# TencentARC/TVTS

Measured on AMD Instinct MI355X. Metric: video-text pairs/sec/node, TVTSv2 pretrain step, higher is better.
Workload: dtype bf16; 1 GPU; TVTSv2 ViT-B/16 8-frame 224^2, mask 0.5, 32-token captions x4, full pretrain step (fwd+losses+bwd+HF-AdamW); pairs_per_gpu=192, global_batch=192, parallelism=dp1, hip_graph=False

## Files before the change

include/tvts_hip.h:

```cpp
#ifndef TVTS_HIP_H
#define TVTS_HIP_H
#include <hip/hip_runtime_api.h>
#ifdef __cplusplus
extern "C" {
#endif

enum { TVTS_ACT_NONE = 0, TVTS_ACT_QUICK_GELU = 1, TVTS_ACT_GELU_ERF = 2,
       TVTS_GATE_ADD_BF16 = 3  };
enum { TVTS_ATTN_FULL = 0, TVTS_ATTN_SPACE = 1, TVTS_ATTN_TIME = 2, TVTS_ATTN_CLS = 3 };
enum {
    TVTS_GEMM_TILE_128 = 1,
    TVTS_GEMM_TILE_256 = 2,
    TVTS_GEMM_FP8_K32 = 4,
    TVTS_TN_NO_EARLY_DMA = 4,
    TVTS_TN_AFAST_0 = 8,
    TVTS_TN_AFAST_1 = 16,
    TVTS_GEMM_STREAMK = 32,
    TVTS_GEMM_NO_STREAMK = 64,
    TVTS_GEMM_RING = 128,
    TVTS_GEMM_NO_RING = 16384,
    TVTS_GEMM_F32_PATCH = 4194304,
    TVTS_GEMM_CLOCK_SAMPLE = 2097152,
    TVTS_GEMM_SIDE_DERIV = 1048576
};
#define TVTS_GEMM_RING_ROWS(r) ((r) == 128 ? (1 << 16) : (r) == 192 ? (2 << 16) : (r) == 256 ? (3 << 16) : 0)
#define TVTS_GEMM_CUS(n) ((((n) / 8) & 63) << 8)
#define TVTS_TN_SPLITS(s) ((s) << 8)
enum {
    TVTS_ATTN_NO_TR = 1,
    TVTS_ATTN_NO_SHARED = 2,
    TVTS_ATTN_NO_FUSED = 4
};

int tvts_gemm_nt_bf16(const void* A, int lda, const void* B, int ldb, int M, int N, int K, const float* bias,
                      const float* residual, int ldr, int act, void* preact, int ldp, const void* gate_h, int ldh,
                      int gate_act, void* out, int ldc, int out_f32, void* workspace, long workspace_bytes, int opts,
                      hipStream_t stream);
long tvts_gemm_nt_workspace_bytes(void);
int tvts_gemm_nt_select(int M, int N, int opts);
int tvts_gemm_tn_bf16(const void* P, int ldp, const void* Q, int ldq, int M, int Na, int Nb, float* out, int ldo,
                      int accumulate, float* colsum, float* workspace, long workspace_elems, int* counters, int n_counters,
                      int opts, hipStream_t stream);
int tvts_gemm_tn_bf16_grouped(const void* problems, int n, void* table_dev, void* table_host, long table_bytes, int upload,
                              float* workspace, long workspace_elems, int opts, hipStream_t stream);
long tvts_gemm_tn_grouped_table_bytes(int n);
int tvts_gemm_tn_select(int M, int Na, int Nb, int opts);
int tvts_gemm_nt_fp8(const void* A, int lda, const void* B, int ldb, int M, int N, int K, const float* scale_a,
                     int scale_a_rows, const float* scale_b, const float* bias, const float* residual, int ldr, int act, void* preact, int ldp,
                     void* out, int ldc, int out_f32, void* q8out, int ldq8, const float* q8_scale, float* q8_amax, int opts,
                     hipStream_t stream);
int tvts_gemm_nt_fp8_gate(const void* A, int lda, const void* B, int ldb, int M, int N, int K, const float* scale_a,
                          int scale_a_rows, const float* scale_b, const float* bias, const void* gate_h, int ldh, int gate_act,
                          void* out, int ldc, void* q8out, int ldq8, const float* q8_scale, float* q8_amax, int opts,
                          hipStream_t stream);
int tvts_gemm_tn_fp8(const void* P8, int ldp, const void* Q8, int ldq, int M, int Na, int Nb, const float* scale_p,
                     const float* scale_q, float* out, int ldo, int accumulate, float* colsum, float* workspace,
                     long workspace_elems, int opts, hipStream_t stream);
int tvts_amax(const void* x, int is_f32, long ld, int rows, int cols, float* amax, hipStream_t stream);
int tvts_quant_fp8(const void* x, int is_f32, long ld, int rows, int cols, const float* amax, void* out, long ldo,
                   float* scale_out, hipStream_t stream);
int tvts_quant_fp8_multi(const void* table, int n, hipStream_t stream);
int tvts_quant_fp8_rows(const void* x, long ld, int rows, int cols, void* out, long ldo, float* row_scale,
                        const float* tscale, float* amax_acc, hipStream_t stream);
int tvts_fp8_update_scales(float* amax, float* scale, int n, hipStream_t stream);
int tvts_gemm_small_f32(const float* A, long sai, long sak, const float* B, long sbk, long sbj, int M, int N, int K,
                        float alpha, const float* bias, float* C, long ldc, int accumulate, hipStream_t stream);
int tvts_rows_linear_bf16(const void* A, long lda, const void* W, int ldw, int R, int N, int K, const float* bias, const float* residual,
                          int ldr, float* out, int ldo, hipStream_t stream);
// ... 187 lines not shown
```

tvts_amd/csrc/gemm.hip:

```cpp
#include "common.h"
#include <stdlib.h>
#include <type_traits>

#include "gemm_nt256.h"

#define BM 128
#define BN 128
#define NTHREADS 256

__device__ __forceinline__ void stage_rows128(const bf16* __restrict__ base, int ld, int row0, int row_max,
                                              int k0, char* lds_tile, int wave, int lane) {
#pragma unroll
    for (int t = 0; t < 4; ++t) {
        const int r0 = (t * 4 + wave) * 8;
        const int row = r0 + (lane >> 3);
        const int slot = lane & 7;
        const int chunk = slot ^ (row & 7);
        int grow = row0 + row;
        grow = grow < row_max ? grow : row_max;
        const bf16* src = base + (size_t)grow * ld + k0 + chunk * 8;
        __builtin_amdgcn_global_load_lds((const GLB_PTR(void))src, (LDS_PTR(void))(lds_tile + r0 * 128), 16, 0, 0);
    }
}

// ... 857 lines not shown
    const int grid = ceil_div(g.n_items, 8) * 8;
    if (t256) {
        hipError_t e2 = hipFuncSetAttribute((const void*)gemm_tn256_kernel, hipFuncAttributeMaxDynamicSharedMemorySize, 131072);
        if (e2 != hipSuccess) return (int)e2;
        hipLaunchKernelGGL(gemm_tn256_kernel, dim3(grid), dim3(512), 131072, stream, g);
    } else {
        hipError_t e2 = hipFuncSetAttribute((const void*)gemm_tn_kernel, hipFuncAttributeMaxDynamicSharedMemorySize, 65536);
        if (e2 != hipSuccess) return (int)e2;
        hipLaunchKernelGGL(gemm_tn_kernel, dim3(grid), dim3(NTHREADS), 65536, stream, g);
    }
    if (use_ws && !fused) {
        const long n4 = (long)Na * Nb / 4;
        int rb = (int)((n4 + 255) / 256);
        if (rb > 2048) rb = 2048;
        hipLaunchKernelGGL(tn_reduce_kernel, dim3(rb), dim3(256), 0, stream, workspace, splits, Na, Nb, out, ldo, accumulate,
                           g.cs_ws, colsum);
    }
    TVTS_LAUNCH_CHECK();
    return TVTS_OK;
}

struct tvts_tn_problem_ { const void* P; int ldp; const void* Q; int ldq; int M, Na, Nb; float* out; int ldo; int accumulate; float* colsum; };
extern "C" long tvts_gemm_tn_grouped_table_bytes(int n) { return (long)n * (long)sizeof(GemmTN) + (long)(n + 1) * 4 + 64; }
extern "C" int tvts_gemm_tn_bf16_grouped(const void* problems, int n, void* table_dev, void* table_host, long table_bytes, int upload,
                                         float* workspace, long workspace_elems, int opts, hipStream_t stream) {
    if (n <= 0 || n > 64 || !problems || !table_dev || !workspace || table_bytes < tvts_gemm_tn_grouped_table_bytes(n)) return TVTS_EINVAL;
    if (upload && !table_host) return TVTS_EINVAL;
    const tvts_tn_problem_* pr = (const tvts_tn_problem_*)problems;
    GemmTN tab_local[64];
    int prefix_local[65];
    GemmTN* tab = upload ? (GemmTN*)table_host : tab_local;
    int* prefix = upload ? (int*)((char*)table_host + (size_t)n * sizeof(GemmTN)) : prefix_local;
    long tiles_total = 0, out_total = 0;
    int Mmax = 0;
    for (int i = 0; i < n; ++i) {
        if (pr[i].M <= 0 || pr[i].Na % 8 || pr[i].Nb % 8 || pr[i].ldp % 8 || pr[i].ldq % 8 || pr[i].ldo % 4 || pr[i].Nb % 4) return TVTS_EINVAL;
        tiles_total += (long)ceil_div(pr[i].Na, 128) * ceil_div(pr[i].Nb, 128);
        out_total += (long)pr[i].Na * pr[i].Nb;
        Mmax = pr[i].M > Mmax ? pr[i].M : Mmax;
    }
    int sp_best = 1;
    if ((opts >> 8) > 0) {
        sp_best = opts >> 8;
    } else {
        double best = 1e30;
        for (int sp = 1; sp <= 32; ++sp) {
            if (sp > 1 && Mmax / sp < 512) break;
            if (sp > 1 && (double)sp * ((double)out_total + 4096.0 * n) > (double)workspace_elems) break;
            const double rounds = (double)((tiles_total * sp + 511) / 512);
            const double t = rounds * (ceil_div(ceil_div(Mmax, sp), 64) * 64.0) * 0.0148 + (sp > 1 ? sp * (double)out_total * 1e-6 : 0.0);
            if (t < best) { best = t; sp_best = sp; }
        }
    }
    float* ws = workspace;
    long used = 0;
    prefix[0] = 0;
    for (int i = 0; i < n; ++i) {
        GemmTN& g = tab[i];
        const tvts_tn_problem_& q = pr[i];
        g.P = (const bf16*)q.P; g.ldp = q.ldp; g.Q = (const bf16*)q.Q; g.ldq = q.ldq; g.M = q.M; g.Na = q.Na; g.Nb = q.Nb;
        g.out = q.out; g.ldo = q.ldo; g.colsum = q.colsum; g.accumulate = q.accumulate; g.cnt = nullptr;
        g.tiles_a = ceil_div(q.Na, 128); g.tiles_b = ceil_div(q.Nb, 128); g.tiles_ab = g.tiles_a * g.tiles_b;
        g.a_fast = g.tiles_a < g.tiles_b ? 1 : 0;
        g.early_dma = ((unsigned long long)q.M * (unsigned long long)(q.ldp > q.ldq ? q.ldp : q.ldq) * 2ull < (1ull << 32)) ? 1 : 0;
        int splits = sp_best;
        while (splits > 1 && q.M / splits < 256) --splits;
        g.m_per_split = ceil_div(ceil_div(q.M, splits), 64) * 64;
        splits = ceil_div(q.M, g.m_per_split);
        g.splits = splits;
        g.ws = nullptr; g.cs_ws = nullptr;
        if (splits > 1) {
            const long need = (long)splits * q.Na * q.Nb + (q.colsum ? (long)splits * q.Na : 0);
            if (used + need > workspace_elems) return TVTS_EINVAL;
            g.ws = ws + used;
            if (q.colsum) g.cs_ws = ws + used + (long)splits * q.Na * q.Nb;
            used += (need + 63) / 64 * 64;
        }
        g.atomic = (q.accumulate || splits > 1) ? 1 : 0;
        g.n_items = g.tiles_ab * splits;
        prefix[i + 1] = prefix[i] + g.n_items;
        if (splits == 1 && !q.accumulate) {  }
    }
    char* td = (char*)table_dev;
    if (upload) {
        hipError_t e = hipMemcpyAsync(td, table_host, (size_t)n * sizeof(GemmTN) + (size_t)(n + 1) * 4, hipMemcpyHostToDevice, stream);
        if (e != hipSuccess) return (int)e;
    }
    TnGroup grp;
    grp.tab = (const GemmTN*)td; grp.prefix = (const int*)(td + (size_t)n * sizeof(GemmTN)); grp.n = n;
    const int grid = ceil_div(prefix[n], 8) * 8;
    hipError_t e2 = hipFuncSetAttribute((const void*)gemm_tn_grouped_kernel, hipFuncAttributeMaxDynamicSharedMemorySize, 65536);
    if (e2 != hipSuccess) return (int)e2;
    hipLaunchKernelGGL(gemm_tn_grouped_kernel, dim3(grid), dim3(NTHREADS), 65536, stream, grp);
    bool any_ws = false;
    for (int i = 0; i < n; ++i) any_ws = any_ws || tab[i].ws != nullptr;
    if (any_ws) hipLaunchKernelGGL(tn_reduce_grouped_kernel, dim3(384, n), dim3(256), 0, stream, grp);
    TVTS_LAUNCH_CHECK();
    return TVTS_OK;
}

#include "gemm_tn8.h"

extern "C" int tvts_gemm_tn_fp8(const void* P8, int ldp, const void* Q8, int ldq, int M, int Na, int Nb, const float* scale_p,
                                const float* scale_q, float* out, int ldo, int accumulate, float* colsum, float* workspace,
                                long workspace_elems, int opts, hipStream_t stream) {
    if (M <= 0 || Na <= 0 || Nb <= 0 || !scale_p || !scale_q) return TVTS_EINVAL;
    if (Na % 16 || Nb % 16 || ldp % 16 || ldq % 16 || ldo % 4) return TVTS_EINVAL;
    if ((unsigned long long)M * (unsigned long long)(ldp > ldq ? ldp : ldq) >= (1ull << 32)) return TVTS_EINVAL;
    GemmTN8 g;
    g.P = (const unsigned char*)P8; g.ldp = ldp; g.Q = (const unsigned char*)Q8; g.ldq = ldq; g.M = M; g.Na = Na; g.Nb = Nb;
    g.out = out; g.ldo = ldo; g.sp = scale_p; g.sq = scale_q; g.accumulate = accumulate; g.ws = nullptr;
    g.colsum = colsum; g.cs_ws = nullptr;
    g.tiles_a = ceil_div(Na, 256); g.tiles_b = ceil_div(Nb, 256); g.tiles_ab = g.tiles_a * g.tiles_b;
    g.a_fast = g.tiles_a < g.tiles_b ? 1 : 0;
    int splits = 1;
    if ((opts >> 8) > 0) {
// ... 349 lines not shown
```

tvts_amd/csrc/gemm_tn256.h:

```cpp
#pragma once

__device__ __forceinline__ unsigned tn_frag_off(int ct, int lane) {
    const int g = lane >> 4, i = lane & 15;
    const int row = g * 4 + (i >> 2);
    return (unsigned)(row * 256 + ((ct ^ (row & 7)) << 5) + (i & 3) * 8);
}
#ifndef TN_STAGGER_DMA
#define TN_STAGGER_DMA 1
#endif
#ifndef TN_ABL
#define TN_ABL 0
#endif
__device__ __forceinline__ bf16x8 tn_frag(const char* tile, unsigned off, int u) {
    typedef __attribute__((ext_vector_type(8))) short s16x8;
    if (TN_ABL & 2) return *(const bf16x8*)(tile + ((off + u * 8192) & ~15u));
    const s16x4 h0 = __builtin_amdgcn_ds_read_tr16_b64_v4i16((LDS_PTR(s16x4))(tile + off + u * 8192));
    const s16x4 h1 = __builtin_amdgcn_ds_read_tr16_b64_v4i16((LDS_PTR(s16x4))(tile + off + u * 8192 + 4096));
    const s16x8 both = __builtin_shufflevector(h0, h1, 0, 1, 2, 3, 4, 5, 6, 7);
    return __builtin_bit_cast(bf16x8, both);
}
__device__ __forceinline__ void tn_mask(bf16x8& f, int u, int valid, int lane) {
    typedef __attribute__((ext_vector_type(4))) unsigned u32x4;
    const int gq = lane >> 4;
    u32x4 w = __builtin_bit_cast(u32x4, f);
// ... 19 lines not shown
                                                       unsigned lds_stage, int wave, int lane) {
    asm volatile("" : "+v"(lane));
#pragma unroll
    for (int q = 0; q < 8; ++q) {
        const int tile = q >> 1;
        const int r0 = ((q & 1) * 8 + wave) * 4;
        const int row = r0 + (lane >> 4);
        const int s16 = lane & 15;
        const int chunk32 = (s16 >> 1) ^ (row & 7);
        const bool isP = tile < 2;
        const int c0 = (isP ? a0 : b0) + (tile & 1) * 128;
        const int cmax = (isP ? g.Na : g.Nb) - 8;
        int col = c0 + chunk32 * 16 + (s16 & 1) * 8;
        col = col < cmax ? col : cmax;
        int gm = m_stage + row;
        gm = gm < g.M - 1 ? gm : g.M - 1;
        const unsigned off = ((unsigned)(gm - m_stage) * (unsigned)(isP ? g.ldp : g.ldq) + (unsigned)col) * 2u;
        glds16_asm(off, isP ? baseP : baseQ, lds_stage + (unsigned)tile * 16384u + (unsigned)r0 * 256u);
    }
}

__global__ __launch_bounds__(512, 2) void gemm_tn256_kernel(GemmTN g) {
    extern __shared__ __attribute__((aligned(16))) char smem[];
    const int tid = threadIdx.x;
    const int lane = tid & 63;
    const int wave = __builtin_amdgcn_readfirstlane(tid >> 6);
    const int wa = wave >> 2, wb = wave & 3;

    const int xcd = blockIdx.x & 7, jx = blockIdx.x >> 3, per = gridDim.x >> 3;
    const int item = xcd * per + jx;
    if (item >= g.n_items) return;
    const int split = item / g.tiles_ab;
    const int t = item % g.tiles_ab;
    const int ta = g.a_fast ? t % g.tiles_a : t / g.tiles_b, tb = g.a_fast ? t / g.tiles_a : t % g.tiles_b;
    const int a0 = ta * 256, b0 = tb * 256;
    const int m_begin = split * g.m_per_split;
    int m_end = m_begin + g.m_per_split;
    m_end = m_end < g.M ? m_end : g.M;
    if (m_begin >= m_end) return;
    const int nk = (m_end - m_begin + 63) / 64;
    const bool do_cs = g.colsum != nullptr && tb == 0;

    const unsigned lds0 = (unsigned)(size_t)(LDS_PTR(char))smem;
    const char* baseP = (const char*)g.P + (size_t)m_begin * g.ldp * 2;
    const char* baseQ = (const char*)g.Q + (size_t)m_begin * g.ldq * 2;
    const size_t stepP = (size_t)64 * g.ldp * 2, stepQ = (size_t)64 * g.ldq * 2;
    const int row_l = wave * 4 + (lane >> 4), s16_l = lane & 15;
    const int col_l = (((s16_l >> 1) ^ (row_l & 7)) << 4) + (s16_l & 1) * 8;
    const unsigned offP = ((unsigned)row_l * (unsigned)g.ldp + (unsigned)(a0 + col_l)) * 2u;
    const unsigned offQ = ((unsigned)row_l * (unsigned)g.ldq + (unsigned)(b0 + col_l)) * 2u;
    const bool cols_inside = a0 + 256 <= g.Na && b0 + 256 <= g.Nb;
    const size_t halfP = (size_t)32 * g.ldp * 2, halfQ = (size_t)32 * g.ldq * 2;
    int i_st = 0;
    auto issue = [&]() {
        const int m_stage = m_begin + i_st * 64;
        const unsigned dst = lds0 + (unsigned)(i_st & 1) * 65536u + (unsigned)wave * 1024u;
        const char* bp = baseP + ((TN_ABL & 4) ? 0 : (size_t)i_st * stepP);
        const char* bq = baseQ + ((TN_ABL & 4) ? 0 : (size_t)i_st * stepQ);
        if (cols_inside && m_stage + 64 <= g.M) {
            glds16_asm_imm<0>(offP, bp, dst);
            glds16_asm_imm<0>(offP, bp + halfP, dst + 8192u);
            glds16_asm_imm<256>(offP, bp, dst + 16384u);
            glds16_asm_imm<256>(offP, bp + halfP, dst + 16384u + 8192u);
            glds16_asm_imm<0>(offQ, bq, dst + 32768u);
            glds16_asm_imm<0>(offQ, bq + halfQ, dst + 32768u + 8192u);
            glds16_asm_imm<256>(offQ, bq, dst + 49152u);
            glds16_asm_imm<256>(offQ, bq + halfQ, dst + 49152u + 8192u);
        } else {
            tn_stage_issue_clamped(g, a0, b0, m_stage, bp, bq, lds0 + (unsigned)(i_st & 1) * 65536u, wave, lane);
        }
        ++i_st;
    };
    issue();
    asm volatile("s_waitcnt vmcnt(0)" ::: "memory");
    RAW_BARRIER_P();
    if (i_st < nk) issue();

    f32x4 acc[8][4];
#pragma unroll
    for (int i = 0; i < 8; ++i)
#pragma unroll
        for (int j = 0; j < 4; ++j) acc[i][j] = (f32x4){0.f, 0.f, 0.f, 0.f};
    float cs0 = 0.f, cs1 = 0.f;

    const unsigned off0 = tn_frag_off(0, lane);
    const unsigned pBase = (unsigned)wa * 16384u, qBase = 32768u + (unsigned)(wb >> 1) * 16384u;
    const unsigned qOff0 = off0 ^ ((unsigned)(wb & 1) << 7);
#define pOff(ct) (pBase + (off0 ^ ((unsigned)(ct) << 5)))
#define qOff(j) (qBase + (qOff0 ^ ((unsigned)(j) << 5)))

    bf16x8 pF[2][4], qF[2][4];
#define TN_LOAD_P(dst, buf, u, h, valid)                                                               \
    _Pragma("unroll") for (int i = 0; i < 4; ++i) {                                                    \
        dst[i] = tn_frag(buf, pOff((h) * 4 + i), u);                                                   \
        if (TAIL && (valid) < 64) tn_mask(dst[i], u, valid, lane);                                     \
    }
#define TN_LOAD_Q(dst, buf, u) _Pragma("unroll") for (int j = 0; j < 4; ++j) dst[j] = tn_frag(buf, qOff(j), u)
#define TN_MFMA16(pv, qv, h)                                                                           \
    _Pragma("unroll") for (int i = 0; i < 4; ++i)                                                      \
        _Pragma("unroll") for (int j = 0; j < 4; ++j)                                                  \
            acc[(h) * 4 + i][j] = __builtin_amdgcn_mfma_f32_16x16x32_bf16(qv[j], pv[i], acc[(h) * 4 + i][j], 0, 0, 0)
#define TN_CS1(acc_, frag_)                                                                            \
    {                                                                                                  \
        typedef __attribute__((ext_vector_type(2))) __bf16 bf16x2_;                                    \
        typedef __attribute__((ext_vector_type(4))) unsigned u32x4_;                                   \
        const u32x4_ w_ = __builtin_bit_cast(u32x4_, frag_);                                           \
        const bf16x2_ one_ = {(bf16)1.0f, (bf16)1.0f};                                                 \
        _Pragma("unroll") for (int d = 0; d < 4; ++d) {                                                \
            const unsigned wd_ = w_[d];                                                                \
            acc_ = __builtin_amdgcn_fdot2_f32_bf16(__builtin_bit_cast(bf16x2_, wd_), one_, acc_, false); \
        }                                                                                              \
    }
#define TN_CS(pv, h)                                                                                   \
    if (CS && (wb >> 1) == (h)) {                                                                      \
        if (wb & 1) { TN_CS1(cs0, pv[2]) TN_CS1(cs1, pv[3]) }                                          \
        else        { TN_CS1(cs0, pv[0]) TN_CS1(cs1, pv[1]) }                                          \
    }
    int valid = m_end - m_begin;
    {
        constexpr bool TAIL = true;
        TN_LOAD_Q(qF[0], smem, 0);
        TN_LOAD_P(pF[0], smem, 0, 0, valid);
    }
#define TN_STAGE()                                                                                     \
    {                                                                                                  \
        const char* cur = smem + (st & 1) * 65536;                                                     \
        const char* nxt = smem + ((st + 1) & 1) * 65536;                                               \
        const int valid_n = valid - 64;                                                                \
        TN_LOAD_P(pF[1], cur, 0, 1, valid);                                                            \
        TN_MFMA16(pF[0], qF[0], 0);                                                                    \
        TN_CS(pF[0], 0);                                                                               \
        TN_LOAD_Q(qF[1], cur, 1);                                                                      \
        TN_LOAD_P(pF[0], cur, 1, 0, valid);                                                            \
        TN_MFMA16(pF[1], qF[0], 1);                                                                    \
        TN_CS(pF[1], 1);                                                                               \
        TN_LOAD_P(pF[1], cur, 1, 1, valid);                                                            \
        TN_MFMA16(pF[0], qF[1], 0);                                                                    \
        TN_CS(pF[0], 0);                                                                               \
        __builtin_amdgcn_s_waitcnt(0x0070);  \
         \
        RAW_BARRIER_P();                                                                               \
         \
         \
         \
        const bool do_issue = i_st < nk && !(TN_ABL & 1);                                              \
        if (do_issue && (!TN_STAGGER_DMA || wave < 4)) issue();                                        \
        if (!TAIL || st + 1 < nk) {        \
            TN_LOAD_Q(qF[0], nxt, 0);                                                                  \
            TN_LOAD_P(pF[0], nxt, 0, 0, valid_n);                                                      \
        }                                                                                              \
        TN_MFMA16(pF[1], qF[1], 1);                                                                    \
        TN_CS(pF[1], 1);                                                                               \
        if (do_issue && TN_STAGGER_DMA && wave >= 4) issue();                                          \
        valid = valid_n;                                                                               \
    }
    int st = 0;
    if (do_cs) {
        constexpr bool CS = true;
        { constexpr bool TAIL = false; for (; st < nk && valid >= 128; ++st) TN_STAGE() }
        { constexpr bool TAIL = true; for (; st < nk; ++st) TN_STAGE() }
    } else {
        constexpr bool CS = false;
        { constexpr bool TAIL = false; for (; st < nk && valid >= 128; ++st) TN_STAGE() }
        { constexpr bool TAIL = true; for (; st < nk; ++st) TN_STAGE() }
    }
#undef TN_STAGE
#undef pOff
#undef qOff
#undef TN_LOAD_P
#undef TN_LOAD_Q
#undef TN_MFMA16
#undef TN_CS
#undef TN_CS1
    if (do_cs) {
        cs0 += __shfl_xor(cs0, 16, 64); cs0 += __shfl_xor(cs0, 32, 64);
        cs1 += __shfl_xor(cs1, 16, 64); cs1 += __shfl_xor(cs1, 32, 64);
        if (lane < 16) {
            const int a = a0 + wa * 128 + 2 * wb * 16 + lane;
            if (a < g.Na) tn_colsum_out(g, split, a, cs0);
            if (a + 16 < g.Na) tn_colsum_out(g, split, a + 16, cs1);
        }
    }
    if (g.cnt) {
        tn_fused_reduce<8, 4>(g, acc, t, split, a0 + wa * 128, b0 + wb * 64, lane, (int*)smem);
        if (*(volatile int*)smem == g.splits - 1 && do_cs && g.cs_ws && lane < 16) {
            const int a = a0 + wa * 128 + 2 * wb * 16 + lane;
            if (a < g.Na) tn_fused_colsum(g, a);
            if (a + 16 < g.Na) tn_fused_colsum(g, a + 16);
        }
        return;
    }
    float* obase = g.ws ? g.ws + (size_t)split * g.Na * g.Nb : g.out;
    const int old_ = g.ws ? g.Nb : g.ldo;
#pragma unroll
    for (int i = 0; i < 8; ++i) {
        const int a = a0 + wa * 128 + i * 16 + (lane & 15);
        if (a >= g.Na) continue;
#pragma unroll
        for (int j = 0; j < 4; ++j) {
            const int b = b0 + wb * 64 + j * 16 + (lane >> 4) * 4;
            if (b >= g.Nb) continue;
            float* dst = obase + (size_t)a * old_ + b;
            if (g.atomic && !g.ws) {
#pragma unroll
                for (int e = 0; e < 4; ++e) atomicAdd(dst + e, acc[i][j][e]);
            } else {
                *(f32x4*)dst = acc[i][j];
            }
        }
    }
}
```

tvts_amd/engine.py:

```python
from __future__ import annotations

import math
from collections import OrderedDict
from typing import Dict, Optional

import numpy as np
import os

import torch

from . import hip as K
from .arch import is_mfma_weight, n_keep, param_shapes, patches_per_frame

CH = 1024


class ParamStore:

    def __init__(self, arch: dict, device: torch.device):
        if arch.get("fp8_wgrad"):
            arch["fp8"] = arch["fp8_dgrad"] = True
        self.arch = arch
        self.device = device
        self.shapes = param_shapes(arch)
# ... 326 lines not shown
                        epi["store_out"] = False
                        self._x8_only.add(q8_for)
            if a8 is None:
                q, sa, kw = self._q8(M, a.shape[1], "x." + wname, persistent=True)
                K.quantize_fp8_rows(a[:M], q=q, **kw)
                a8 = (q, sa)
            self._x8[wname] = a8
            K.gemm_nt_fp8(a8[0], a8[1], w8, ws, out[:M], bias=self.P.p(bname) if bname else None, **epi)
            return
        K.gemm_nt(a, self.P.w(wname), out, M=M, bias=self.P.p(bname) if bname else None, **epi)

    def _cls_lin(self, a, S, wname, bname, res_c, out_c, fwd_only=False):
        Bc = out_c.shape[0]
        if wname in self._x8_only and not fwd_only:
            q, sa = self._x8[wname]
            w8, ws, _ = self.P.w8[wname]
            K.gemm_nt_fp8(q[:Bc * S].view(Bc, -1)[:, :q.shape[1]], sa, w8, ws, out_c, bias=self.P.p(bname) if bname else None, residual=res_c)
            return
        a_c = a[:Bc * S].view(Bc, -1)[:, :a.shape[1]]
        K.rows_linear(a_c, self.P.w(wname), out_c, bias=self.P.p(bname) if bname else None, residual=res_c)

    TN_GROUPED_MIN_ROWS, TN_GROUPED_MAX_ROWS = 6000, 12000

    def _tn_grouped_on(self, M) -> bool:
        on = self.tn_grouped
        if on is None:
            on = self.TN_GROUPED_MIN_ROWS <= M <= self.TN_GROUPED_MAX_ROWS
        return bool(on) and not self.fp8_wgrad and not self.wgrad_stream

    def _tn_group_run(self, key, problems):
        if not problems:
            return
        sig = tuple((pr["p"].data_ptr(), pr["q"].data_ptr(), pr["out"].data_ptr(), pr["M"],
                     pr["colsum"].data_ptr() if pr["colsum"] is not None else 0) for pr in problems)
        plans = self._tn_groups.setdefault(key, {})
        grp = plans.get(sig)
        if grp is None:
            if self._tn_group_ws is None:
                self._tn_group_ws = torch.empty(64 * 1024 * 1024, dtype=torch.float32, device=self.dev)
            if len(plans) >= self.TN_GROUP_PLANS_PER_BLOCK:
                old = next((k for k, g in plans.items() if not g.captured), None)
                if old is not None:
                    plans.pop(old)
            grp = plans[sig] = K.TnGroup(problems, self._tn_group_ws, splits=int(self.arch.get("tn_group_splits", 0)))
        grp.run()

    TN_GROUP_PLANS_PER_BLOCK = 4

    def _lin_bwd(self, dy, a_in, wname, bname, d_in, M, dy8=None, side=False, q8_for=None, defer=None, **epi):
        want_b = bool(bname) and self.requires_grad[bname]
        if epi.get("gate_h") is not None and epi.get("gate_act") not in (None, "add") and self.gate_deriv:
            epi["side_deriv"] = True
        f8w = self.fp8_wgrad and self._f8_tensor_mode and wname in self.P.w8t and wname in self._x8
        if dy8 is None:
            dy8 = self._dy8_ready.pop(wname, None)
        if (f8w or (d_in is not None and wname in self.P.w8t)) and dy8 is None:
            q, sa, kw = self._q8(M, dy.shape[1], "dy." + wname)
            K.quantize_fp8_rows(dy[:M], q=q, **kw)
            dy8 = (q, sa)
        if self.requires_grad[wname]:
            if defer is not None and not f8w:
                defer.append(dict(p=dy, q=a_in, out=self.P.g2d(wname), M=M, accumulate=True, colsum=self.P.g(bname) if want_b else None))
            elif f8w:
                x8 = self._x8[wname]
                K.gemm_tn_fp8(dy8[0], dy8[1], x8[0], x8[1], self.P.g2d(wname), M=M, accumulate=True,
                              colsum=self.P.g(bname) if want_b else None)
            elif side:
                ws, scratch = self._side()
# ... 849 lines not shown
```

tvts_amd/hip.py:

```python
from __future__ import annotations

import ctypes
import os
from typing import Optional

import torch

from . import _lib

GEMM_PROFILE = None
HBM_PROFILE = None


class _hbm:

    def __init__(self, family, nbytes):
        self.family, self.nbytes = family, nbytes

    def __enter__(self):
        if HBM_PROFILE is not None:
            self.e0, self.e1 = Event(), Event()
            self.e0.record()

    def __exit__(self, *exc):
# ... 319 lines not shown
    cnt = _tn_counters(ws) if ws is not None else None
    if GEMM_PROFILE is not None:
        ev0, ev1 = Event(), Event()
        ev0.record()
    def launch(fu):
        return lib.tvts_gemm_tn_bf16(_p(p), _ld(p), _p(q), _ld(q), M, p.shape[1], q.shape[1], _p(out), _ld(out),
                                     1 if accumulate else 0, _p(colsum), _p(ws), ws.numel() if ws is not None else 0,
                                     _p(cnt), cnt.numel() if cnt is not None else 0,
                                     tn_opts(tile, splits, early_dma, a_fast, fu), _stream())
    want_fu = _OPTS["tn_streamk"] if fused is None else fused
    rc = launch(fused)
    if rc == -22 and want_fu and fused is None:
        rc = launch(False)
    elif rc == 0 and want_fu:
        STREAMK_TAKEN[0] += 1
    _chk(rc, "tvts_gemm_tn_bf16")
    if GEMM_PROFILE is not None:
        ev1.record()
        GEMM_PROFILE.append(("gemm_tn", 2.0 * M * p.shape[1] * q.shape[1], ev0, ev1, (M, p.shape[1], q.shape[1], "cs" if colsum is not None else "")))


class TnGroup:

    class _Rec(ctypes.Structure):
        _fields_ = [("P", ctypes.c_void_p), ("ldp", ctypes.c_int), ("Q", ctypes.c_void_p), ("ldq", ctypes.c_int), ("M", ctypes.c_int),
                    ("Na", ctypes.c_int), ("Nb", ctypes.c_int), ("out", ctypes.c_void_p), ("ldo", ctypes.c_int),
                    ("accumulate", ctypes.c_int), ("colsum", ctypes.c_void_p)]

    def __init__(self, problems, workspace, splits=0):
        lib = _lib.load()
        self.n = len(problems)
        self.keep = problems
        self.recs = (self._Rec * self.n)()
        for r, pr in zip(self.recs, problems):
            p, q, out = pr["p"], pr["q"], pr["out"]
            assert p.dtype == torch.bfloat16 and q.dtype == torch.bfloat16 and out.dtype == torch.float32
            r.P, r.ldp, r.Q, r.ldq = p.data_ptr(), _ld(p), q.data_ptr(), _ld(q)
            r.M, r.Na, r.Nb = int(pr.get("M") or p.shape[0]), p.shape[1], q.shape[1]
            r.out, r.ldo, r.accumulate = out.data_ptr(), _ld(out), 1 if pr.get("accumulate", True) else 0
            r.colsum = pr["colsum"].data_ptr() if pr.get("colsum") is not None else None
        self.key = tuple((r.P, r.Q, r.out, r.colsum, r.M, r.Na, r.Nb, r.ldp, r.ldq, r.ldo, r.accumulate) for r in self.recs)
        self.ws = workspace
        nbytes = lib.tvts_gemm_tn_grouped_table_bytes(self.n)
        self.table = torch.empty(nbytes, dtype=torch.uint8, device=workspace.device)
        self.table_host = torch.empty(nbytes, dtype=torch.uint8, pin_memory=True)
        self.uploaded = False
        self.captured = False
        self.opts = int(splits) << 8
        self.flops = sum(2.0 * r.M * r.Na * r.Nb for r in self.recs)

    def run(self):
        lib = _lib.load()
        if GEMM_PROFILE is not None:
            ev0, ev1 = Event(), Event()
            ev0.record()
        capturing = torch.cuda.is_current_stream_capturing()
        rc = lib.tvts_gemm_tn_bf16_grouped(ctypes.cast(self.recs, ctypes.c_void_p), self.n, _p(self.table), ctypes.c_void_p(self.table_host.data_ptr()),
                                           self.table.numel(), 0 if (self.uploaded and not capturing) else 1, _p(self.ws), self.ws.numel(), self.opts, _stream())
        _chk(rc, "tvts_gemm_tn_bf16_grouped")
        if capturing:
            self.captured = True
        else:
            self.uploaded = True
        if GEMM_PROFILE is not None:
            ev1.record()
            r0 = self.recs[0]
            GEMM_PROFILE.append(("gemm_tn", self.flops, ev0, ev1, (r0.M, sum(r.Na * r.Nb for r in self.recs) // max(r0.Nb, 1), r0.Nb, "grouped")))


def gemm_tn_fp8(p8, sp, q8, sq, out, *, M=None, accumulate=True, colsum=None, workspace=True, splits=None):
    lib = _lib.load()
# ... 614 lines not shown
```

Baseline: 1404 pairs/s.

## Add 256-tile grouped TN weight-gradient GEMM path for very large row counts

```diff
diff --git a/include/tvts_hip.h b/include/tvts_hip.h
--- a/include/tvts_hip.h
+++ b/include/tvts_hip.h
@@ -44,6 +44,7 @@
 int tvts_gemm_tn_bf16_grouped(const void* problems, int n, void* table_dev, void* table_host, long table_bytes, int upload,
                               float* workspace, long workspace_elems, int opts, hipStream_t stream);
 long tvts_gemm_tn_grouped_table_bytes(int n);
+long tvts_gemm_tn_grouped_workspace_elems(const void* problems, int n, int opts);
 int tvts_gemm_tn_select(int M, int Na, int Nb, int opts);
 int tvts_gemm_nt_fp8(const void* A, int lda, const void* B, int ldb, int M, int N, int K, const float* scale_a,
                      int scale_a_rows, const float* scale_b, const float* bias, const float* residual, int ldr, int act, void* preact, int ldp,
diff --git a/tvts_amd/csrc/gemm.hip b/tvts_amd/csrc/gemm.hip
--- a/tvts_amd/csrc/gemm.hip
+++ b/tvts_amd/csrc/gemm.hip
@@ -903,6 +903,75 @@
 
 struct tvts_tn_problem_ { const void* P; int ldp; const void* Q; int ldq; int M, Na, Nb; float* out; int ldo; int accumulate; float* colsum; };
 extern "C" long tvts_gemm_tn_grouped_table_bytes(int n) { return (long)n * (long)sizeof(GemmTN) + (long)(n + 1) * 4 + 64; }
+
+static bool tn_group_use_256(const tvts_tn_problem_* pr, int n, int opts) {
+    for (int i = 0; i < n; ++i)
+        if (!tn_use_256(pr[i].M, pr[i].Na, pr[i].Nb, opts)) return false;
+    return true;
+}
+static void tn_group_ranges_256(const tvts_tn_problem_& q, int opts, int* m_per_split, int* splits) {
+    int sp = (opts >> 8) > 0 ? (opts >> 8) : tn_best_splits(q.M, q.Na, q.Nb, 256, nullptr);
+    *m_per_split = ceil_div(ceil_div(q.M, sp), 64) * 64;
+    *splits = ceil_div(q.M, *m_per_split);
+}
+static long tn_group_ws_need(const tvts_tn_problem_& q, int splits) {
+    if (splits <= 1) return 0;
+    const long need = (long)splits * q.Na * q.Nb + (q.colsum ? (long)splits * q.Na : 0);
+    return (need + 63) / 64 * 64;
+}
+extern "C" long tvts_gemm_tn_grouped_workspace_elems(const void* problems, int n, int opts) {
+    if (n <= 0 || n > 64 || !problems) return TVTS_EINVAL;
+    const tvts_tn_problem_* pr = (const tvts_tn_problem_*)problems;
+    for (int i = 0; i < n; ++i)
+        if (pr[i].M <= 0 || pr[i].Na <= 0 || pr[i].Nb <= 0) return TVTS_EINVAL;
+    if (!tn_group_use_256(pr, n, opts)) return 0;
+    long total = 0;
+    for (int i = 0; i < n; ++i) {
+        int mps, sp;
+        tn_group_ranges_256(pr[i], opts, &mps, &sp);
+        total += tn_group_ws_need(pr[i], sp);
+    }
+    return total;
+}
+static int tn_grouped_256(const tvts_tn_problem_* pr, int n, GemmTN* tab, int* prefix, float* workspace, long workspace_elems, int opts) {
+    int order[64];
+    int mps[64], sps[64];
+    for (int i = 0; i < n; ++i) {
+        order[i] = i;
+        tn_group_ranges_256(pr[i], opts, &mps[i], &sps[i]);
+    }
+    for (int i = 1; i < n; ++i) {
+        const int o = order[i];
+        int j = i;
+        for (; j > 0 && mps[order[j - 1]] < mps[o]; --j) order[j] = order[j - 1];
+        order[j] = o;
+    }
+    long used = 0;
+    prefix[0] = 0;
+    for (int k = 0; k < n; ++k) {
+        GemmTN& g = tab[k];
+        const tvts_tn_problem_& q = pr[order[k]];
+        g.P = (const bf16*)q.P; g.ldp = q.ldp; g.Q = (const bf16*)q.Q; g.ldq = q.ldq; g.M = q.M; g.Na = q.Na; g.Nb = q.Nb;
+        g.out = q.out; g.ldo = q.ldo; g.colsum = q.colsum; g.accumulate = q.accumulate; g.cnt = nullptr;
+        g.tiles_a = ceil_div(q.Na, 256); g.tiles_b = ceil_div(q.Nb, 256); g.tiles_ab = g.tiles_a * g.tiles_b;
+        g.a_fast = (opts & 8) ? 0 : (opts & 16) ? 1 : (g.tiles_a < g.tiles_b ? 1 : 0);
+        g.early_dma = 0;
+        g.m_per_split = mps[order[k]];
+        g.splits = sps[order[k]];
+        g.ws = nullptr; g.cs_ws = nullptr;
+        if (g.splits > 1) {
+            const long need = tn_group_ws_need(q, g.splits);
+            if (used + need > workspace_elems) return TVTS_EINVAL;
+            g.ws = workspace + used;
+            if (q.colsum) g.cs_ws = workspace + used + (long)g.splits * q.Na * q.Nb;
+            used += need;
+        }
+        g.atomic = (q.accumulate || g.splits > 1) ? 1 : 0;
+        g.n_items = g.tiles_ab * g.splits;
+        prefix[k + 1] = prefix[k] + ceil_div(g.n_items, 8);
+    }
+    return TVTS_OK;
+}
 extern "C" int tvts_gemm_tn_bf16_grouped(const void* problems, int n, void* table_dev, void* table_host, long table_bytes, int upload,
                                          float* workspace, long workspace_elems, int opts, hipStream_t stream) {
     if (n <= 0 || n > 64 || !problems || !table_dev || !workspace || table_bytes < tvts_gemm_tn_grouped_table_bytes(n)) return TVTS_EINVAL;
@@ -920,6 +989,11 @@
         out_total += (long)pr[i].Na * pr[i].Nb;
         Mmax = pr[i].M > Mmax ? pr[i].M : Mmax;
     }
+    const bool t256 = tn_group_use_256(pr, n, opts);
+    if (t256) {
+        const int rc = tn_grouped_256(pr, n, tab, prefix, workspace, workspace_elems, opts);
+        if (rc != TVTS_OK) return rc;
+    }
     int sp_best = 1;
     if ((opts >> 8) > 0) {
         sp_best = opts >> 8;
@@ -936,7 +1010,7 @@
     float* ws = workspace;
     long used = 0;
     prefix[0] = 0;
-    for (int i = 0; i < n; ++i) {
+    for (int i = 0; i < n && !t256; ++i) {
         GemmTN& g = tab[i];
         const tvts_tn_problem_& q = pr[i];
         g.P = (const bf16*)q.P; g.ldp = q.ldp; g.Q = (const bf16*)q.Q; g.ldq = q.ldq; g.M = q.M; g.Na = q.Na; g.Nb = q.Nb;
@@ -969,10 +1043,16 @@
     }
     TnGroup grp;
     grp.tab = (const GemmTN*)td; grp.prefix = (const int*)(td + (size_t)n * sizeof(GemmTN)); grp.n = n;
-    const int grid = ceil_div(prefix[n], 8) * 8;
-    hipError_t e2 = hipFuncSetAttribute((const void*)gemm_tn_grouped_kernel, hipFuncAttributeMaxDynamicSharedMemorySize, 65536);
-    if (e2 != hipSuccess) return (int)e2;
-    hipLaunchKernelGGL(gemm_tn_grouped_kernel, dim3(grid), dim3(NTHREADS), 65536, stream, grp);
+    if (t256) {
+        hipError_t e2 = hipFuncSetAttribute((const void*)gemm_tn256_grouped_kernel, hipFuncAttributeMaxDynamicSharedMemorySize, 131072);
+        if (e2 != hipSuccess) return (int)e2;
+        hipLaunchKernelGGL(gemm_tn256_grouped_kernel, dim3(prefix[n] * 8), dim3(512), 131072, stream, grp);
+    } else {
+        const int grid = ceil_div(prefix[n], 8) * 8;
+        hipError_t e2 = hipFuncSetAttribute((const void*)gemm_tn_grouped_kernel, hipFuncAttributeMaxDynamicSharedMemorySize, 65536);
+        if (e2 != hipSuccess) return (int)e2;
+        hipLaunchKernelGGL(gemm_tn_grouped_kernel, dim3(grid), dim3(NTHREADS), 65536, stream, grp);
+    }
     bool any_ws = false;
     for (int i = 0; i < n; ++i) any_ws = any_ws || tab[i].ws != nullptr;
     if (any_ws) hipLaunchKernelGGL(tn_reduce_grouped_kernel, dim3(384, n), dim3(256), 0, stream, grp);
diff --git a/tvts_amd/csrc/gemm_tn256.h b/tvts_amd/csrc/gemm_tn256.h
--- a/tvts_amd/csrc/gemm_tn256.h
+++ b/tvts_amd/csrc/gemm_tn256.h
@@ -65,191 +65,19 @@
 
 __global__ __launch_bounds__(512, 2) void gemm_tn256_kernel(GemmTN g) {
     extern __shared__ __attribute__((aligned(16))) char smem[];
-    const int tid = threadIdx.x;
-    const int lane = tid & 63;
-    const int wave = __builtin_amdgcn_readfirstlane(tid >> 6);
-    const int wa = wave >> 2, wb = wave & 3;
-
     const int xcd = blockIdx.x & 7, jx = blockIdx.x >> 3, per = gridDim.x >> 3;
     const int item = xcd * per + jx;
-    if (item >= g.n_items) return;
-    const int split = item / g.tiles_ab;
-    const int t = item % g.tiles_ab;
-    const int ta = g.a_fast ? t % g.tiles_a : t / g.tiles_b, tb = g.a_fast ? t / g.tiles_a : t % g.tiles_b;
-    const int a0 = ta * 256, b0 = tb * 256;
-    const int m_begin = split * g.m_per_split;
-    int m_end = m_begin + g.m_per_split;
-    m_end = m_end < g.M ? m_end : g.M;
-    if (m_begin >= m_end) return;
-    const int nk = (m_end - m_begin + 63) / 64;
-    const bool do_cs = g.colsum != nullptr && tb == 0;
+#include "gemm_tn256_item.h"
+}
 
-    const unsigned lds0 = (unsigned)(size_t)(LDS_PTR(char))smem;
-    const char* baseP = (const char*)g.P + (size_t)m_begin * g.ldp * 2;
-    const char* baseQ = (const char*)g.Q + (size_t)m_begin * g.ldq * 2;
-    const size_t stepP = (size_t)64 * g.ldp * 2, stepQ = (size_t)64 * g.ldq * 2;
-    const int row_l = wave * 4 + (lane >> 4), s16_l = lane & 15;
-    const int col_l = (((s16_l >> 1) ^ (row_l & 7)) << 4) + (s16_l & 1) * 8;
-    const unsigned offP = ((unsigned)row_l * (unsigned)g.ldp + (unsigned)(a0 + col_l)) * 2u;
-    const unsigned offQ = ((unsigned)row_l * (unsigned)g.ldq + (unsigned)(b0 + col_l)) * 2u;
-    const bool cols_inside = a0 + 256 <= g.Na && b0 + 256 <= g.Nb;
-    const size_t halfP = (size_t)32 * g.ldp * 2, halfQ = (size_t)32 * g.ldq * 2;
-    int i_st = 0;
-    auto issue = [&]() {
-        const int m_stage = m_begin + i_st * 64;
-        const unsigned dst = lds0 + (unsigned)(i_st & 1) * 65536u + (unsigned)wave * 1024u;
-        const char* bp = baseP + ((TN_ABL & 4) ? 0 : (size_t)i_st * stepP);
-        const char* bq = baseQ + ((TN_ABL & 4) ? 0 : (size_t)i_st * stepQ);
-        if (cols_inside && m_stage + 64 <= g.M) {
-            glds16_asm_imm<0>(offP, bp, dst);
-            glds16_asm_imm<0>(offP, bp + halfP, dst + 8192u);
-            glds16_asm_imm<256>(offP, bp, dst + 16384u);
-            glds16_asm_imm<256>(offP, bp + halfP, dst + 16384u + 8192u);
-            glds16_asm_imm<0>(offQ, bq, dst + 32768u);
-            glds16_asm_imm<0>(offQ, bq + halfQ, dst + 32768u + 8192u);
-            glds16_asm_imm<256>(offQ, bq, dst + 49152u);
-            glds16_asm_imm<256>(offQ, bq + halfQ, dst + 49152u + 8192u);
-        } else {
-            tn_stage_issue_clamped(g, a0, b0, m_stage, bp, bq, lds0 + (unsigned)(i_st & 1) * 65536u, wave, lane);
-        }
-        ++i_st;
-    };
-    issue();
-    asm volatile("s_waitcnt vmcnt(0)" ::: "memory");
-    RAW_BARRIER_P();
-    if (i_st < nk) issue();
-
-    f32x4 acc[8][4];
-#pragma unroll
-    for (int i = 0; i < 8; ++i)
-#pragma unroll
-        for (int j = 0; j < 4; ++j) acc[i][j] = (f32x4){0.f, 0.f, 0.f, 0.f};
-    float cs0 = 0.f, cs1 = 0.f;
-
-    const unsigned off0 = tn_frag_off(0, lane);
-    const unsigned pBase = (unsigned)wa * 16384u, qBase = 32768u + (unsigned)(wb >> 1) * 16384u;
-    const unsigned qOff0 = off0 ^ ((unsigned)(wb & 1) << 7);
-#define pOff(ct) (pBase + (off0 ^ ((unsigned)(ct) << 5)))
-#define qOff(j) (qBase + (qOff0 ^ ((unsigned)(j) << 5)))
-
-    bf16x8 pF[2][4], qF[2][4];
-#define TN_LOAD_P(dst, buf, u, h, valid)                                                               \
-    _Pragma("unroll") for (int i = 0; i < 4; ++i) {                                                    \
-        dst[i] = tn_frag(buf, pOff((h) * 4 + i), u);                                                   \
-        if (TAIL && (valid) < 64) tn_mask(dst[i], u, valid, lane);                                     \
-    }
-#define TN_LOAD_Q(dst, buf, u) _Pragma("unroll") for (int j = 0; j < 4; ++j) dst[j] = tn_frag(buf, qOff(j), u)
-#define TN_MFMA16(pv, qv, h)                                                                           \
-    _Pragma("unroll") for (int i = 0; i < 4; ++i)                                                      \
-        _Pragma("unroll") for (int j = 0; j < 4; ++j)                                                  \
-            acc[(h) * 4 + i][j] = __builtin_amdgcn_mfma_f32_16x16x32_bf16(qv[j], pv[i], acc[(h) * 4 + i][j], 0, 0, 0)
-#define TN_CS1(acc_, frag_)                                                                            \
-    {                                                                                                  \
-        typedef __attribute__((ext_vector_type(2))) __bf16 bf16x2_;                                    \
-        typedef __attribute__((ext_vector_type(4))) unsigned u32x4_;                                   \
-        const u32x4_ w_ = __builtin_bit_cast(u32x4_, frag_);                                           \
-        const bf16x2_ one_ = {(bf16)1.0f, (bf16)1.0f};                                                 \
-        _Pragma("unroll") for (int d = 0; d < 4; ++d) {                                                \
-            const unsigned wd_ = w_[d];                                                                \
-            acc_ = __builtin_amdgcn_fdot2_f32_bf16(__builtin_bit_cast(bf16x2_, wd_), one_, acc_, false); \
-        }                                                                                              \
-    }
-#define TN_CS(pv, h)                                                                                   \
-    if (CS && (wb >> 1) == (h)) {                                                                      \
-        if (wb & 1) { TN_CS1(cs0, pv[2]) TN_CS1(cs1, pv[3]) }                                          \
-        else        { TN_CS1(cs0, pv[0]) TN_CS1(cs1, pv[1]) }                                          \
-    }
-    int valid = m_end - m_begin;
-    {
-        constexpr bool TAIL = true;
-        TN_LOAD_Q(qF[0], smem, 0);
-        TN_LOAD_P(pF[0], smem, 0, 0, valid);
-    }
-#define TN_STAGE()                                                                                     \
-    {                                                                                                  \
-        const char* cur = smem + (st & 1) * 65536;                                                     \
-        const char* nxt = smem + ((st + 1) & 1) * 65536;                                               \
-        const int valid_n = valid - 64;                                                                \
-        TN_LOAD_P(pF[1], cur, 0, 1, valid);                                                            \
-        TN_MFMA16(pF[0], qF[0], 0);                                                                    \
-        TN_CS(pF[0], 0);                                                                               \
-        TN_LOAD_Q(qF[1], cur, 1);                                                                      \
-        TN_LOAD_P(pF[0], cur, 1, 0, valid);                                                            \
-        TN_MFMA16(pF[1], qF[0], 1);                                                                    \
-        TN_CS(pF[1], 1);                                                                               \
-        TN_LOAD_P(pF[1], cur, 1, 1, valid);                                                            \
-        TN_MFMA16(pF[0], qF[1], 0);                                                                    \
-        TN_CS(pF[0], 0);                                                                               \
-        __builtin_amdgcn_s_waitcnt(0x0070);  \
-         \
-        RAW_BARRIER_P();                                                                               \
-         \
-         \
-         \
-        const bool do_issue = i_st < nk && !(TN_ABL & 1);                                              \
-        if (do_issue && (!TN_STAGGER_DMA || wave < 4)) issue();                                        \
-        if (!TAIL || st + 1 < nk) {        \
-            TN_LOAD_Q(qF[0], nxt, 0);                                                                  \
-            TN_LOAD_P(pF[0], nxt, 0, 0, valid_n);                                                      \
-        }                                                                                              \
-        TN_MFMA16(pF[1], qF[1], 1);                                                                    \
-        TN_CS(pF[1], 1);                                                                               \
-        if (do_issue && TN_STAGGER_DMA && wave >= 4) issue();                                          \
-        valid = valid_n;                                                                               \
-    }
-    int st = 0;
-    if (do_cs) {
-        constexpr bool CS = true;
-        { constexpr bool TAIL = false; for (; st < nk && valid >= 128; ++st) TN_STAGE() }
-        { constexpr bool TAIL = true; for (; st < nk; ++st) TN_STAGE() }
-    } else {
-        constexpr bool CS = false;
-        { constexpr bool TAIL = false; for (; st < nk && valid >= 128; ++st) TN_STAGE() }
-        { constexpr bool TAIL = true; for (; st < nk; ++st) TN_STAGE() }
-    }
-#undef TN_STAGE
-#undef pOff
-#undef qOff
-#undef TN_LOAD_P
-#undef TN_LOAD_Q
-#undef TN_MFMA16
-#undef TN_CS
-#undef TN_CS1
-    if (do_cs) {
-        cs0 += __shfl_xor(cs0, 16, 64); cs0 += __shfl_xor(cs0, 32, 64);
-        cs1 += __shfl_xor(cs1, 16, 64); cs1 += __shfl_xor(cs1, 32, 64);
-        if (lane < 16) {
-            const int a = a0 + wa * 128 + 2 * wb * 16 + lane;
-            if (a < g.Na) tn_colsum_out(g, split, a, cs0);
-            if (a + 16 < g.Na) tn_colsum_out(g, split, a + 16, cs1);
-        }
-    }
-    if (g.cnt) {
-        tn_fused_reduce<8, 4>(g, acc, t, split, a0 + wa * 128, b0 + wb * 64, lane, (int*)smem);
-        if (*(volatile int*)smem == g.splits - 1 && do_cs && g.cs_ws && lane < 16) {
-            const int a = a0 + wa * 128 + 2 * wb * 16 + lane;
-            if (a < g.Na) tn_fused_colsum(g, a);
-            if (a + 16 < g.Na) tn_fused_colsum(g, a + 16);
-        }
-        return;
-    }
-    float* obase = g.ws ? g.ws + (size_t)split * g.Na * g.Nb : g.out;
-    const int old_ = g.ws ? g.Nb : g.ldo;
-#pragma unroll
-    for (int i = 0; i < 8; ++i) {
-        const int a = a0 + wa * 128 + i * 16 + (lane & 15);
-        if (a >= g.Na) continue;
-#pragma unroll
-        for (int j = 0; j < 4; ++j) {
-            const int b = b0 + wb * 64 + j * 16 + (lane >> 4) * 4;
-            if (b >= g.Nb) continue;
-            float* dst = obase + (size_t)a * old_ + b;
-            if (g.atomic && !g.ws) {
-#pragma unroll
-                for (int e = 0; e < 4; ++e) atomicAdd(dst + e, acc[i][j][e]);
-            } else {
-                *(f32x4*)dst = acc[i][j];
-            }
-        }
-    }
+__global__ __launch_bounds__(512, 2) void gemm_tn256_grouped_kernel(TnGroup grp) {
+    extern __shared__ __attribute__((aligned(16))) char smem[];
+    const int xcd = blockIdx.x & 7, jx = blockIdx.x >> 3;
+    if (jx >= grp.prefix[grp.n]) return;
+    int p = 0;
+    while (p + 1 < grp.n && jx >= grp.prefix[p + 1]) ++p;
+    const GemmTN g = grp.tab[p];
+    const int first = grp.prefix[p], per = grp.prefix[p + 1] - first;
+    const int item = xcd * per + (jx - first);
+#include "gemm_tn256_item.h"
 }
diff --git a/tvts_amd/csrc/gemm_tn256_item.h b/tvts_amd/csrc/gemm_tn256_item.h
--- /dev/null
+++ b/tvts_amd/csrc/gemm_tn256_item.h
@@ -0,0 +1,184 @@
+    const int tid = threadIdx.x;
+    const int lane = tid & 63;
+    const int wave = __builtin_amdgcn_readfirstlane(tid >> 6);
+    const int wa = wave >> 2, wb = wave & 3;
+    if (item >= g.n_items) return;
+    const int split = item / g.tiles_ab;
+    const int t = item % g.tiles_ab;
+    const int ta = g.a_fast ? t % g.tiles_a : t / g.tiles_b, tb = g.a_fast ? t / g.tiles_a : t % g.tiles_b;
+    const int a0 = ta * 256, b0 = tb * 256;
+    const int m_begin = split * g.m_per_split;
+    int m_end = m_begin + g.m_per_split;
+    m_end = m_end < g.M ? m_end : g.M;
+    if (m_begin >= m_end) return;
+    const int nk = (m_end - m_begin + 63) / 64;
+    const bool do_cs = g.colsum != nullptr && tb == 0;
+
+    const unsigned lds0 = (unsigned)(size_t)(LDS_PTR(char))smem;
+    const char* baseP = (const char*)g.P + (size_t)m_begin * g.ldp * 2;
+    const char* baseQ = (const char*)g.Q + (size_t)m_begin * g.ldq * 2;
+    const size_t stepP = (size_t)64 * g.ldp * 2, stepQ = (size_t)64 * g.ldq * 2;
+    const int row_l = wave * 4 + (lane >> 4), s16_l = lane & 15;
+    const int col_l = (((s16_l >> 1) ^ (row_l & 7)) << 4) + (s16_l & 1) * 8;
+    const unsigned offP = ((unsigned)row_l * (unsigned)g.ldp + (unsigned)(a0 + col_l)) * 2u;
+    const unsigned offQ = ((unsigned)row_l * (unsigned)g.ldq + (unsigned)(b0 + col_l)) * 2u;
+    const bool cols_inside = a0 + 256 <= g.Na && b0 + 256 <= g.Nb;
+    const size_t halfP = (size_t)32 * g.ldp * 2, halfQ = (size_t)32 * g.ldq * 2;
+    int i_st = 0;
+    auto issue = [&]() {
+        const int m_stage = m_begin + i_st * 64;
+        const unsigned dst = lds0 + (unsigned)(i_st & 1) * 65536u + (unsigned)wave * 1024u;
+        const char* bp = baseP + ((TN_ABL & 4) ? 0 : (size_t)i_st * stepP);
+        const char* bq = baseQ + ((TN_ABL & 4) ? 0 : (size_t)i_st * stepQ);
+        if (cols_inside && m_stage + 64 <= g.M) {
+            glds16_asm_imm<0>(offP, bp, dst);
+            glds16_asm_imm<0>(offP, bp + halfP, dst + 8192u);
+            glds16_asm_imm<256>(offP, bp, dst + 16384u);
+            glds16_asm_imm<256>(offP, bp + halfP, dst + 16384u + 8192u);
+            glds16_asm_imm<0>(offQ, bq, dst + 32768u);
+            glds16_asm_imm<0>(offQ, bq + halfQ, dst + 32768u + 8192u);
+            glds16_asm_imm<256>(offQ, bq, dst + 49152u);
+            glds16_asm_imm<256>(offQ, bq + halfQ, dst + 49152u + 8192u);
+        } else {
+            tn_stage_issue_clamped(g, a0, b0, m_stage, bp, bq, lds0 + (unsigned)(i_st & 1) * 65536u, wave, lane);
+        }
+        ++i_st;
+    };
+    issue();
+    asm volatile("s_waitcnt vmcnt(0)" ::: "memory");
+    RAW_BARRIER_P();
+    if (i_st < nk) issue();
+
+    f32x4 acc[8][4];
+#pragma unroll
+    for (int i = 0; i < 8; ++i)
+#pragma unroll
+        for (int j = 0; j < 4; ++j) acc[i][j] = (f32x4){0.f, 0.f, 0.f, 0.f};
+    float cs0 = 0.f, cs1 = 0.f;
+
+    const unsigned off0 = tn_frag_off(0, lane);
+    const unsigned pBase = (unsigned)wa * 16384u, qBase = 32768u + (unsigned)(wb >> 1) * 16384u;
+    const unsigned qOff0 = off0 ^ ((unsigned)(wb & 1) << 7);
+#define pOff(ct) (pBase + (off0 ^ ((unsigned)(ct) << 5)))
+#define qOff(j) (qBase + (qOff0 ^ ((unsigned)(j) << 5)))
+
+    bf16x8 pF[2][4], qF[2][4];
+#define TN_LOAD_P(dst, buf, u, h, valid)                                                               \
+    _Pragma("unroll") for (int i = 0; i < 4; ++i) {                                                    \
+        dst[i] = tn_frag(buf, pOff((h) * 4 + i), u);                                                   \
+        if (TAIL && (valid) < 64) tn_mask(dst[i], u, valid, lane);                                     \
+    }
+#define TN_LOAD_Q(dst, buf, u) _Pragma("unroll") for (int j = 0; j < 4; ++j) dst[j] = tn_frag(buf, qOff(j), u)
+#define TN_MFMA16(pv, qv, h)                                                                           \
+    _Pragma("unroll") for (int i = 0; i < 4; ++i)                                                      \
+        _Pragma("unroll") for (int j = 0; j < 4; ++j)                                                  \
+            acc[(h) * 4 + i][j] = __builtin_amdgcn_mfma_f32_16x16x32_bf16(qv[j], pv[i], acc[(h) * 4 + i][j], 0, 0, 0)
+#define TN_CS1(acc_, frag_)                                                                            \
+    {                                                                                                  \
+        typedef __attribute__((ext_vector_type(2))) __bf16 bf16x2_;                                    \
+        typedef __attribute__((ext_vector_type(4))) unsigned u32x4_;                                   \
+        const u32x4_ w_ = __builtin_bit_cast(u32x4_, frag_);                                           \
+        const bf16x2_ one_ = {(bf16)1.0f, (bf16)1.0f};                                                 \
+        _Pragma("unroll") for (int d = 0; d < 4; ++d) {                                                \
+            const unsigned wd_ = w_[d];                                                                \
+            acc_ = __builtin_amdgcn_fdot2_f32_bf16(__builtin_bit_cast(bf16x2_, wd_), one_, acc_, false); \
+        }                                                                                              \
+    }
+#define TN_CS(pv, h)                                                                                   \
+    if (CS && (wb >> 1) == (h)) {                                                                      \
+        if (wb & 1) { TN_CS1(cs0, pv[2]) TN_CS1(cs1, pv[3]) }                                          \
+        else        { TN_CS1(cs0, pv[0]) TN_CS1(cs1, pv[1]) }                                          \
+    }
+    int valid = m_end - m_begin;
+    {
+        constexpr bool TAIL = true;
+        TN_LOAD_Q(qF[0], smem, 0);
+        TN_LOAD_P(pF[0], smem, 0, 0, valid);
+    }
+#define TN_STAGE()                                                                                     \
+    {                                                                                                  \
+        const char* cur = smem + (st & 1) * 65536;                                                     \
+        const char* nxt = smem + ((st + 1) & 1) * 65536;                                               \
+        const int valid_n = valid - 64;                                                                \
+        TN_LOAD_P(pF[1], cur, 0, 1, valid);                                                            \
+        TN_MFMA16(pF[0], qF[0], 0);                                                                    \
+        TN_CS(pF[0], 0);                                                                               \
+        TN_LOAD_Q(qF[1], cur, 1);                                                                      \
+        TN_LOAD_P(pF[0], cur, 1, 0, valid);                                                            \
+        TN_MFMA16(pF[1], qF[0], 1);                                                                    \
+        TN_CS(pF[1], 1);                                                                               \
+        TN_LOAD_P(pF[1], cur, 1, 1, valid);                                                            \
+        TN_MFMA16(pF[0], qF[1], 0);                                                                    \
+        TN_CS(pF[0], 0);                                                                               \
+        __builtin_amdgcn_s_waitcnt(0x0070);  \
+         \
+        RAW_BARRIER_P();                                                                               \
+         \
+         \
+         \
+        const bool do_issue = i_st < nk && !(TN_ABL & 1);                                              \
+        if (do_issue && (!TN_STAGGER_DMA || wave < 4)) issue();                                        \
+        if (!TAIL || st + 1 < nk) {        \
+            TN_LOAD_Q(qF[0], nxt, 0);                                                                  \
+            TN_LOAD_P(pF[0], nxt, 0, 0, valid_n);                                                      \
+        }                                                                                              \
+        TN_MFMA16(pF[1], qF[1], 1);                                                                    \
+        TN_CS(pF[1], 1);                                                                               \
+        if (do_issue && TN_STAGGER_DMA && wave >= 4) issue();                                          \
+        valid = valid_n;                                                                               \
+    }
+    int st = 0;
+    if (do_cs) {
+        constexpr bool CS = true;
+        { constexpr bool TAIL = false; for (; st < nk && valid >= 128; ++st) TN_STAGE() }
+        { constexpr bool TAIL = true; for (; st < nk; ++st) TN_STAGE() }
+    } else {
+        constexpr bool CS = false;
+        { constexpr bool TAIL = false; for (; st < nk && valid >= 128; ++st) TN_STAGE() }
+        { constexpr bool TAIL = true; for (; st < nk; ++st) TN_STAGE() }
+    }
+#undef TN_STAGE
+#undef pOff
+#undef qOff
+#undef TN_LOAD_P
+#undef TN_LOAD_Q
+#undef TN_MFMA16
+#undef TN_CS
+#undef TN_CS1
+    if (do_cs) {
+        cs0 += __shfl_xor(cs0, 16, 64); cs0 += __shfl_xor(cs0, 32, 64);
+        cs1 += __shfl_xor(cs1, 16, 64); cs1 += __shfl_xor(cs1, 32, 64);
+        if (lane < 16) {
+            const int a = a0 + wa * 128 + 2 * wb * 16 + lane;
+            if (a < g.Na) tn_colsum_out(g, split, a, cs0);
+            if (a + 16 < g.Na) tn_colsum_out(g, split, a + 16, cs1);
+        }
+    }
+    if (g.cnt) {
+        tn_fused_reduce<8, 4>(g, acc, t, split, a0 + wa * 128, b0 + wb * 64, lane, (int*)smem);
+        if (*(volatile int*)smem == g.splits - 1 && do_cs && g.cs_ws && lane < 16) {
+            const int a = a0 + wa * 128 + 2 * wb * 16 + lane;
+            if (a < g.Na) tn_fused_colsum(g, a);
+            if (a + 16 < g.Na) tn_fused_colsum(g, a + 16);
+        }
+        return;
+    }
+    float* obase = g.ws ? g.ws + (size_t)split * g.Na * g.Nb : g.out;
+    const int old_ = g.ws ? g.Nb : g.ldo;
+#pragma unroll
+    for (int i = 0; i < 8; ++i) {
+        const int a = a0 + wa * 128 + i * 16 + (lane & 15);
+        if (a >= g.Na) continue;
+#pragma unroll
+        for (int j = 0; j < 4; ++j) {
+            const int b = b0 + wb * 64 + j * 16 + (lane >> 4) * 4;
+            if (b >= g.Nb) continue;
+            float* dst = obase + (size_t)a * old_ + b;
+            if (g.atomic && !g.ws) {
+#pragma unroll
+                for (int e = 0; e < 4; ++e) atomicAdd(dst + e, acc[i][j][e]);
+            } else {
+                *(f32x4*)dst = acc[i][j];
+            }
+        }
+    }
diff --git a/tvts_amd/engine.py b/tvts_amd/engine.py
--- a/tvts_amd/engine.py
+++ b/tvts_amd/engine.py
@@ -372,10 +372,15 @@
 
     TN_GROUPED_MIN_ROWS, TN_GROUPED_MAX_ROWS = 6000, 12000
 
+    TN_GROUPED_BIG_ROWS = 150000
+
     def _tn_grouped_on(self, M) -> bool:
         on = self.tn_grouped
         if on is None:
             on = self.TN_GROUPED_MIN_ROWS <= M <= self.TN_GROUPED_MAX_ROWS
+            if not on and M >= self.TN_GROUPED_BIG_ROWS:
+                W = self.arch["width"]
+                on = all(K.gemm_tn_select(M, na, nb) == 256 for na, nb in ((W, W), (3 * W, W), (4 * W, W), (W, 4 * W)))
         return bool(on) and not self.fp8_wgrad and not self.wgrad_stream
 
     def _tn_group_run(self, key, problems):
@@ -386,14 +391,17 @@
         plans = self._tn_groups.setdefault(key, {})
         grp = plans.get(sig)
         if grp is None:
-            if self._tn_group_ws is None:
-                self._tn_group_ws = torch.empty(64 * 1024 * 1024, dtype=torch.float32, device=self.dev)
             if len(plans) >= self.TN_GROUP_PLANS_PER_BLOCK:
                 old = next((k for k, g in plans.items() if not g.captured), None)
                 if old is not None:
                     plans.pop(old)
-            grp = plans[sig] = K.TnGroup(problems, self._tn_group_ws, splits=int(self.arch.get("tn_group_splits", 0)))
+            grp = plans[sig] = K.TnGroup(problems, self._tn_group_scratch, splits=int(self.arch.get("tn_group_splits", 0)))
         grp.run()
+
+    def _tn_group_scratch(self, elems):
+        if self._tn_group_ws is None or self._tn_group_ws.numel() < elems:
+            self._tn_group_ws = torch.empty(elems, dtype=torch.float32, device=self.dev)
+        return self._tn_group_ws
 
     TN_GROUP_PLANS_PER_BLOCK = 4
 
diff --git a/tvts_amd/hip.py b/tvts_amd/hip.py
--- a/tvts_amd/hip.py
+++ b/tvts_amd/hip.py
@@ -365,12 +365,14 @@
 
 class TnGroup:
 
+    MIN_WORKSPACE = 64 * 1024 * 1024
+
     class _Rec(ctypes.Structure):
         _fields_ = [("P", ctypes.c_void_p), ("ldp", ctypes.c_int), ("Q", ctypes.c_void_p), ("ldq", ctypes.c_int), ("M", ctypes.c_int),
                     ("Na", ctypes.c_int), ("Nb", ctypes.c_int), ("out", ctypes.c_void_p), ("ldo", ctypes.c_int),
                     ("accumulate", ctypes.c_int), ("colsum", ctypes.c_void_p)]
 
-    def __init__(self, problems, workspace, splits=0):
+    def __init__(self, problems, workspace=None, splits=0, tile=None):
         lib = _lib.load()
         self.n = len(problems)
         self.keep = problems
@@ -383,13 +385,22 @@
             r.out, r.ldo, r.accumulate = out.data_ptr(), _ld(out), 1 if pr.get("accumulate", True) else 0
             r.colsum = pr["colsum"].data_ptr() if pr.get("colsum") is not None else None
         self.key = tuple((r.P, r.Q, r.out, r.colsum, r.M, r.Na, r.Nb, r.ldp, r.ldq, r.ldo, r.accumulate) for r in self.recs)
+        tile = _OPTS["tn_tile"] if tile is None else tile
+        self.opts = _tile_bits(tile) | (int(splits or _OPTS["tn_splits"]) << 8)
+        self.ws_need = int(lib.tvts_gemm_tn_grouped_workspace_elems(ctypes.cast(self.recs, ctypes.c_void_p), self.n, self.opts))
+        if self.ws_need < 0:
+            _chk(self.ws_need, "tvts_gemm_tn_grouped_workspace_elems")
+        self.tile = 256 if all(lib.tvts_gemm_tn_select(r.M, r.Na, r.Nb, self.opts) == 256 for r in self.recs) else 128
+        if workspace is None:
+            workspace = torch.empty(max(self.ws_need, self.MIN_WORKSPACE), dtype=torch.float32, device=problems[0]["p"].device)
+        elif callable(workspace):
+            workspace = workspace(max(self.ws_need, self.MIN_WORKSPACE))
         self.ws = workspace
         nbytes = lib.tvts_gemm_tn_grouped_table_bytes(self.n)
         self.table = torch.empty(nbytes, dtype=torch.uint8, device=workspace.device)
         self.table_host = torch.empty(nbytes, dtype=torch.uint8, pin_memory=True)
         self.uploaded = False
         self.captured = False
-        self.opts = int(splits) << 8
         self.flops = sum(2.0 * r.M * r.Na * r.Nb for r in self.recs)
 
     def run(self):
```

Measured after the change: 1417 pairs/s (median of 6 runs). No clear change (+0.9%).
